# victorca25/traiNNer

Measured on AMD Instinct MI355X. Metric: HR images/sec (G+D step), ESRGAN x4 128->512, higher is better.
Workload: dtype f32 (bf16x3)

## Files before the change

trainner_amd/csrc/conv_sweep.hip:

```cpp
#include <stddef.h>
#include <string.h>
#include <type_traits>
#include <utility>
#include "conv_body.h"
#include "conv_epilogue.h"
#include "conv_handoff.h"

namespace {

constexpr int SW_TH = 8, SW_TW = 32, SW_HT = SW_TH + 2, SW_WT = SW_TW + 2;
constexpr int SW_ROW = TNR_X3_ROW;
constexpr int SW_A_ROWS = SW_HT * SW_WT;
constexpr int SW_A_ALLOC_ROWS = 384;
constexpr int SW_A_FLOATS = SW_A_ALLOC_ROWS * SW_ROW;
constexpr int SW_UNIT_FLOATS = 32 * SW_ROW;
constexpr int SW_SLOT_UNITS = 9;
constexpr int SW_SLOT_FLOATS = SW_SLOT_UNITS * SW_UNIT_FLOATS;
constexpr int SW_RING = 3;
constexpr size_t SW_LDS_BYTES = (size_t)(2 * SW_A_FLOATS + SW_RING * SW_SLOT_FLOATS) * sizeof(float);
constexpr int SW_NPASS = 9, SW_NSTAGE = 5, SW_NTILE = 6;
constexpr int SW_A_IT = (SW_A_ROWS * 4 + 511) / 512;
constexpr int SW_B_PIECES = (SW_SLOT_UNITS * 3 + 7) / 8;
static_assert(SW_LDS_BYTES <= 160 * 1024, "one sweep workgroup per CU");

// ... 773 lines not shown
            constexpr int S = decltype(sc)::value;
            SW_T(t_e0);
            const ConvK a = sweep_stage(S);
            const __amdgpu_buffer_rsrc_t y_rs =
                __builtin_amdgcn_make_buffer_rsrc(a.y, 0, (int)((unsigned)a.N * a.Ho * a.Wo * a.y_ct * 4u), 0x00020000);
            if constexpr (S < 4) {
                f32x16 t[2][1];
                t[0][0] = acc[0][S];
                t[1][0] = acc[1][S];
                conv_epilogue_dpp<TNR_CONV_3x3, SW_TW, 1, 2, true, 8, false>(a, t, 0, n, ty0, tx0, 0, wave, li, half, y_rs);
            } else {
                f32x16 t[2][2];
#pragma unroll
                for (int m = 0; m < 2; ++m) {
                    t[m][0] = acc[m][4];
                    t[m][1] = acc[m][5];
                }
                conv_epilogue_dpp<TNR_CONV_3x3, SW_TW, 2, 2, true, 8>(a, t, 0, n, ty0, tx0, 0, wave, li, half, y_rs);
            }
            pend_tile = tile;
            pend_value = c.base + (unsigned)S + 1u;
            pend_age = 0;
            { SW_T(t_e1); SW_ADD(8, t_e1 - t_e0); }
        };
        auto sync = [&](auto sc) __attribute__((always_inline)) {
            constexpr int sl = decltype(sc)::value;
            slot_sync((sl + 1) % SW_RING);
        };
        auto item_step = [&](auto ic, auto kc) __attribute__((always_inline)) {
            if (has_next) item_step_buf(ic, kc, (e + 1) & 1);
        };

        sw_static_for<0, P::NPASS>([&](auto pc) __attribute__((always_inline)) {
            constexpr int p = decltype(pc)::value;
            const int nchunks = sw_nchunks(p, c.nck0), ch_lo = sw_ch_lo(p, c.nck0);
#pragma unroll 1
            for (int ck = 0; ck < nchunks; ++ck) {
                slot_sync(1);
                if constexpr (!sw_apass(p) && !(DIRECT && S4D_EPI_AFTER)) {
                    if (ck == 0) epilogue_of(std::integral_constant<int, sw_phase(p)>{});
                }
                const bool last_ck = ck + 1 == nchunks;
                has_next = !(last_ck && p == P::NPASS - 1);
                int ch_keep = 0;
                if (has_next) {
                    int ch_next = ch_lo + 16 * (ck + 1);
                    if (last_ck) {
                        ch_next = sw_ch_lo(p + 1 < P::NPASS ? p + 1 : p, c.nck0);
                        if constexpr (p + 1 < P::NPASS && sw_apass(p + 1)) {
                            const ChainWait w{c.progress, c.base + (unsigned)sw_phase(p + 1), n, ty, tx, c.tiles_x, c.tiles_y, c.err,
                                              &pend_tile, pend_value};
                            SW_T(t_w0);
                            w();
                            { SW_T(t_w1); SW_ADD(1, t_w1 - t_w0); }
                        }
                    }
                    if constexpr (!(DIRECT && S4D_ALOAD_ALWAYS)) {
                        SW_T(t_al0);
                        a_load(ch_next);
                        { SW_T(t_al1); SW_ADD(2, t_al1 - t_al0); }
                    } else {
                        ch_keep = ch_next;
                    }
                }
                if constexpr (DIRECT && S4D_ALOAD_ALWAYS) {
                    SW_T(t_al0);
                    a_load(ch_keep, has_next);
                    { SW_T(t_al1); SW_ADD(2, t_al1 - t_al0); }
                }
                const float *sa = s_a + (e & 1) * SW_A_FLOATS;
                SW_T(t_c0);
                if constexpr (AMP) {
                    auto item1 = [&](auto ic) __attribute__((always_inline)) {
                        if (has_next) a_item1(ic, (e + 1) & 1);
                    };
                    amp4_chunk<P::j0(p), P::nj(p)>(acc, sa, apix0, half, item1, fbq, b_fetch1);
                } else {
                    sweep4_chunk<P::j0(p), P::nj(p), DIRECT>(acc, sa, s_b_lane, apix0, half, sync, item_step, dma_step, tick, fbr, b_fetch);
                }
                { SW_T(t_c1); SW_ADD(6, t_c1 - t_c0); SW_ADD(15, 1ull); SW_ADD(9 + (P::nj(p) == 3 ? 0 : (P::nj(p) == 2 ? 1 : 2)), t_c1 - t_c0); }
                ++e;
            }
            if constexpr (DIRECT && S4D_EPI_AFTER && sw_apass(p) && p + 1 < P::NPASS) {
                epilogue_of(std::integral_constant<int, sw_phase(p)>{});
            }
        });
        epilogue_of(std::integral_constant<int, P::NSTAGE - 1>{});
    }
    asm volatile("s_waitcnt vmcnt(0)" ::: "memory");
    __syncthreads();
    if (pend_tile >= 0 && tid == 0) __hip_atomic_store(c.progress + pend_tile, pend_value, __ATOMIC_RELAXED, __HIP_MEMORY_SCOPE_AGENT);
    if (tid == 0 && atomicAdd(c.disp + 8, 1u) == (unsigned)g - 1u) {
#pragma unroll
        for (int i = 0; i < 9; ++i) __hip_atomic_store(c.disp + i, 0u, __ATOMIC_RELAXED, __HIP_MEMORY_SCOPE_AGENT);
    }
#ifdef SW_TIMELINE
    if (tid == 0) {
        tl[14] = __builtin_amdgcn_s_memtime() - tl_begin;
        for (int i = 0; i < 16; ++i) atomicAdd(&sw_tl[i], tl[i]);
        for (int i = 0; i < 16; ++i) atomicAdd(&sw_tl2[i], tl2[i]);
    }
#endif
}

struct D4K {
    ConvK a;
    const float *wq;
    int wq_bytes;
    int nck;
    int tiles_x, tiles_y, ncb, tiles;
};

struct D4PackK {
    const float *wp;
    int KinP, KoutP, nck, ncb, units;
    int shuffle;
    float *out;
};

__global__ void __launch_bounds__(256) d4_pack_kernel(const D4PackK a) {
    const int g = blockIdx.x * 256 + threadIdx.x;
    const int unit = g >> 6, r = (g >> 1) & 31, h = g & 1;
    if (unit >= a.units) return;
    const int per_cb = a.nck * 18;
    const int cb = unit / per_cb, rem = unit - cb * per_cb;
    const int ck = rem / 18, tj = rem - ck * 18, tap = tj >> 1, j = tj & 1;
    int co = cb * 64 + j * 32 + r;
    if (a.shuffle == 2) {
        const int nfc = a.KoutP >> 2;
        co = (co % nfc) * 4 + co / nfc;
    }
    const float *src = a.wp + ((size_t)tap * a.KoutP + co) * a.KinP + 16 * ck + 8 * h;
    const f32x4 q0 = *reinterpret_cast<const f32x4 *>(src), q1 = *reinterpret_cast<const f32x4 *>(src + 4);
    tnr_bf16x8 pl[3];
    tnr_split_bf16x3(q0, q1, pl);
    float *dst = a.out + (size_t)unit * SW_UNIT_FLOATS + (h * 32 + r) * 4;
#pragma unroll
    for (int k = 0; k < 3; ++k) *reinterpret_cast<tnr_bf16x8 *>(dst + k * 256) = pl[k];
}

template <int OCC, bool AMP = false, bool PS = false>
__global__ void __launch_bounds__(256, OCC) conv3x3_d4_kernel(const D4K c) {
    extern __shared__ __attribute__((aligned(16))) float smem[];
    float *s_a = smem;
    const int tid = threadIdx.x;
    const int wave = __builtin_amdgcn_readfirstlane(tid >> 6), lane = tid & 63, li = lane & 31, half = lane >> 5;
    const ConvK &a = c.a;
    const __amdgpu_buffer_rsrc_t x_rs =
        __builtin_amdgcn_make_buffer_rsrc(const_cast<float *>(a.x), 0, (int)((unsigned)a.N * a.H * a.W * a.x_ct * 4u), 0x00020000);
    const __amdgpu_buffer_rsrc_t w_rs = __builtin_amdgcn_make_buffer_rsrc(const_cast<float *>(c.wq), 0, c.wq_bytes, 0x00020000);
    const __amdgpu_buffer_rsrc_t y_rs =
        __builtin_amdgcn_make_buffer_rsrc(a.y, 0, (int)((unsigned)a.N * a.Ho * a.Wo * a.y_ct * 4u), 0x00020000);
    const int apix0[2] = {(2 * wave) * SW_WT + li, (2 * wave + 1) * SW_WT + li};

    for (int tile = blockIdx.x; tile < c.tiles; tile += gridDim.x) {
        const int cb = tile % c.ncb;
        int rest = tile / c.ncb;
        const int tx = rest % c.tiles_x;
        rest /= c.tiles_x;
        const int ty = rest % c.tiles_y, n = rest / c.tiles_y;
        const int ty0 = ty * SW_TH, tx0 = tx * SW_TW;
        int in_off[S4_A_IT], a_dst[S4_A_IT];
#pragma unroll
        for (int it = 0; it < S4_A_IT; ++it) {
            const int i = tid + it * 256, row = i >> 2, q = i & 3;
            const int hr = row / SW_WT, hc = row - hr * SW_WT;
            int Y = ty0 + hr - 1, X = tx0 + hc - 1;
            if (a.reflect) {
                Y = Y == -1 ? 1 : (Y == a.H ? a.H - 2 : Y);
                X = X == -1 ? 1 : (X == a.W ? a.W - 2 : X);
            }
            const bool in = (row < SW_A_ROWS) & (Y >= 0) & (Y < a.H) & (X >= 0) & (X < a.W);
            in_off[it] = in ? (((n * a.H + Y) * a.W + X) * a.x_ct + a.x_co + q * 4) : -1;
            a_dst[it] = row * SW_ROW + 4 * ((q >> 1) ^ ((row >> TNR_X3_SWZ) & 1)) + 2 * (q & 1);
        }
        f32x4 rin[S4_A_IT];
        auto a_load = [&](int ch, bool valid) __attribute__((always_inline)) {
#pragma unroll
            for (int it = 0; it < S4_A_IT; ++it) {
                const unsigned bo = (valid && in_off[it] >= 0) ? (unsigned)(in_off[it] + ch) * 4u : 0xfffffff0u;
                rin[it] = __builtin_bit_cast(f32x4, __builtin_amdgcn_raw_buffer_load_b128(x_rs, (int)bo, 0, 0));
            }
        };
        tnr_bf16x4 ih, im, il;
        f32x4 ir;
        auto item_step_buf = [&](auto ic, auto kc, int buf) __attribute__((always_inline)) {
            constexpr int it = decltype(ic)::value, k = decltype(kc)::value;
            if constexpr (k == 0) {
                tnr_pk_level(rin[it], ih, ir);
            } else if constexpr (k == 1) {
                const f32x4 r1 = ir;
                tnr_pk_level(r1, im, ir);
            } else {
                if constexpr (k == 2) {
                    const tnr_f32x2 a2 = {ir[0], ir[1]}, b2 = {ir[2], ir[3]};
                    il = __builtin_bit_cast(tnr_bf16x4, tnr_f32x2{__builtin_bit_cast(float, __builtin_convertvector(a2, tnr_bf16x2)),
                                                                __builtin_bit_cast(float, __builtin_convertvector(b2, tnr_bf16x2))});
                }
                float *dst = s_a + buf * SW_A_FLOATS + a_dst[it] + 8 * (k - 2);
                *reinterpret_cast<tnr_f32x2 *>(dst) = __builtin_bit_cast(tnr_f32x2, k == 2 ? ih : (k == 3 ? im : il));
            }
        };
        f32x16 acc[2][SW_NTILE];
#pragma unroll
        for (int m = 0; m < 2; ++m)
#pragma unroll
            for (int j = 0; j < 2; ++j)
#pragma unroll
                for (int r = 0; r < 16; ++r) acc[m][j][r] = 0.f;

        a_load(0, true);
        __syncthreads();
        tnr_bf16x8 fbr[3][3];
        int bq = cb * c.nck * 18;
        auto b_fetch = [&](auto rc, int sp) __attribute__((always_inline)) {
            constexpr int r = decltype(rc)::value;
            fbr[r][sp] = __builtin_bit_cast(tnr_bf16x8, __builtin_amdgcn_raw_buffer_load_b128(w_rs, lane * 16, (bq * 3 + sp) * 1024, 0));
            if (sp == 2) ++bq;
        };
        tnr_bf16x8 fbq[9];
        auto b_fetch1 = [&](auto rc) __attribute__((always_inline)) {
            constexpr int r = decltype(rc)::value;
            fbq[r] = __builtin_bit_cast(tnr_bf16x8, __builtin_amdgcn_raw_buffer_load_b128(w_rs, lane * 16, bq * 3072, 0));
            ++bq;
        };
        auto a_item1 = [&](auto ic, int buf) __attribute__((always_inline)) {
            constexpr int it = decltype(ic)::value;
            const tnr_bf16x4 h = __builtin_convertvector(rin[it], tnr_bf16x4);
            *reinterpret_cast<tnr_f32x2 *>(s_a + buf * SW_A_FLOATS + a_dst[it]) = __builtin_bit_cast(tnr_f32x2, h);
        };
        if constexpr (AMP) {
            sw_static_for<0, 8>([&](auto rc) __attribute__((always_inline)) { b_fetch1(rc); });
            sw_static_for<0, S4_A_IT>([&](auto ic) __attribute__((always_inline)) { a_item1(ic, 0); });
        } else {
#pragma unroll
            for (int sp = 0; sp < 3; ++sp) b_fetch(std::integral_constant<int, 0>{}, sp);
#pragma unroll
            for (int sp = 0; sp < 3; ++sp) b_fetch(std::integral_constant<int, 1>{}, sp);
            sw_static_for<0, S4_A_IT>([&](auto ic) __attribute__((always_inline)) {
                sw_static_for<0, 5>([&](auto kc) __attribute__((always_inline)) { item_step_buf(ic, kc, 0); });
            });
        }
        bool has_next = false;
        int e = 0;
        auto item_step = [&](auto ic, auto kc) __attribute__((always_inline)) {
            if (has_next) item_step_buf(ic, kc, (e + 1) & 1);
        };
        auto nop1 = [&](auto) __attribute__((always_inline)) {};
        auto nop0 = [&]() __attribute__((always_inline)) {};
        auto tick = [&](int, unsigned long long) __attribute__((always_inline)) {};
#pragma unroll 1
        for (int ck = 0; ck < c.nck; ++ck) {
            asm volatile("s_waitcnt lgkmcnt(0)\n\ts_barrier" ::: "memory");
            has_next = ck + 1 < c.nck;
            a_load(16 * (ck + 1), has_next);
            if constexpr (AMP) {
                auto item1 = [&](auto ic) __attribute__((always_inline)) {
                    if (has_next) a_item1(ic, (e + 1) & 1);
                };
                amp4_chunk<0, 2>(acc, s_a + (e & 1) * SW_A_FLOATS, apix0, half, item1, fbq, b_fetch1);
            } else {
                sweep4_chunk<0, 2, true>(acc, s_a + (e & 1) * SW_A_FLOATS, nullptr, apix0, half, nop1, item_step, nop0, tick, fbr, b_fetch);
            }
            ++e;
        }
        f32x16 t[2][2];
#pragma unroll
        for (int m = 0; m < 2; ++m) {
            t[m][0] = acc[m][0];
            t[m][1] = acc[m][1];
        }
        if constexpr (PS) {
            ConvK ap = a;
            const int nfb = c.ncb >> 2, sub = cb / nfb;
            ap.Cout = a.Cout >> 2;
            ap.Ho = 2 * a.Ho;
            ap.Wo = 2 * a.Wo;
            ap.bias = a.bias != nullptr ? a.bias + sub : nullptr;
            conv_epilogue_dpp<TNR_DGRAD_4x4_S2, SW_TW, 2, 2, false, (OCC == 1 ? 8 : 1), false, 4>(ap, t, cb - sub * nfb, n, ty0, tx0, sub, wave, li, half, y_rs);
        } else {
            conv_epilogue_dpp<TNR_CONV_3x3, SW_TW, 2, 2, false, (OCC == 1 ? 8 : 1)>(a, t, cb, n, ty0, tx0, 0, wave, li, half, y_rs);
        }
    }
}

constexpr int S2_TAPS = 4, S2_NU = S2_TAPS * 2, S2_RING = 4;
struct S2K {
    ConvK a;
    const float *wq;
    int wq_bytes;
    int nck;
    int tiles_x, tiles_y, ncb, tiles;
};
struct S2PackK {
    const float *wp;
    int KinP, KoutP, nck, ncb, units, dgrad;
    float *out;
};

__global__ void __launch_bounds__(256) s2_pack_kernel(const S2PackK a) {
    const int g = blockIdx.x * 256 + threadIdx.x;
    const int unit = g >> 6, r = (g >> 1) & 31, h = g & 1;
    if (unit >= a.units) return;
    const int j = unit & 1, tap = (unit >> 1) & 3;
    int rest = unit >> 3;
    const float *src;
    if (a.dgrad) {
        const int ck = rest % a.nck;
        rest /= a.nck;
        const int cb = rest % a.ncb, par = rest / a.ncb;
        src = a.wp + (((size_t)par * 4 + tap) * a.KoutP + cb * 64 + j * 32 + r) * a.KinP + 16 * ck + 8 * h;
    } else {
        const int ck = rest % a.nck;
        rest /= a.nck;
        const int pp = rest & 3, cb = rest >> 2;
        src = a.wp + ((size_t)tap * a.KoutP + cb * 64 + j * 32 + r) * (4 * a.KinP) + pp * a.KinP + 16 * ck + 8 * h;
    }
    const f32x4 q0 = *reinterpret_cast<const f32x4 *>(src), q1 = *reinterpret_cast<const f32x4 *>(src + 4);
    tnr_bf16x8 pl[3];
    tnr_split_bf16x3(q0, q1, pl);
    float *dst = a.out + (size_t)unit * SW_UNIT_FLOATS + (h * 32 + r) * 4;
#pragma unroll
    for (int k = 0; k < 3; ++k) *reinterpret_cast<tnr_bf16x8 *>(dst + k * 256) = pl[k];
}

template <bool AMP, class Item, class BFetch>
__device__ __forceinline__ void tap4_chunk(f32x16 (&acc)[2][2], const float *sa, const int (&aaddr)[2][4], Item &&item_step,
                                           tnr_bf16x8 (&fbr)[S2_RING][3], BFetch &&b_fetch) {
    constexpr int TA[6] = {0, 2, 1, 0, 1, 0}, TB[6] = {2, 0, 1, 1, 0, 0};
    tnr_bf16x8 fa[2][2][3];
    auto read_a = [&](auto tc, int m, int sp) __attribute__((always_inline)) {
        constexpr int t = decltype(tc)::value;
        fa[t & 1][m][sp] = *reinterpret_cast<const tnr_bf16x8 *>(sa + aaddr[m][t] + 8 * sp);
    };
#pragma unroll
    for (int k = 0; k < (AMP ? 2 : 6); ++k) read_a(std::integral_constant<int, 0>{}, AMP ? k : k / 3, AMP ? 0 : k % 3);
    sw_static_for<0, S2_NU>([&](auto uc) __attribute__((always_inline)) {
        constexpr int u = decltype(uc)::value, t = u >> 1, jj = u & 1;
        constexpr bool NEXT_TAP = jj == 1 && t + 1 < S2_TAPS;
        constexpr int ITEM = u - (S2_NU - 6);
        __builtin_amdgcn_sched_barrier(0);
        if constexpr (AMP) {
            sw_static_for<0, 2>([&](auto mc) __attribute__((always_inline)) {
                constexpr int m = decltype(mc)::value;
                acc[m][jj] = __builtin_amdgcn_mfma_f32_32x32x16_bf16(fa[t & 1][m][0], fbr[u % S2_RING][0], acc[m][jj], 0, 0, 0);
                if constexpr (m == 0) b_fetch(std::integral_constant<int, (u + 3) % S2_RING>{}, 0);
                if constexpr (NEXT_TAP) read_a(std::integral_constant<int, (t + 1 < S2_TAPS ? t + 1 : t)>{}, m, 0);
                if constexpr (m == 1 && ITEM >= 0) item_step(std::integral_constant<int, (ITEM >= 0 ? ITEM : 0)>{}, std::integral_constant<int, -1>{});
                __builtin_amdgcn_sched_barrier(0);
            });
        } else {
            sw_static_for<0, 12>([&](auto ic) __attribute__((always_inline)) {
                constexpr int i = decltype(ic)::value, p = i / 2, m = i % 2;
                acc[m][jj] = __builtin_amdgcn_mfma_f32_32x32x16_bf16(fa[t & 1][m][TA[p]], fbr[u % S2_RING][TB[p]], acc[m][jj], 0, 0, 0);
                if constexpr (i < 3) b_fetch(std::integral_constant<int, (u + 3) % S2_RING>{}, i);
                if constexpr (NEXT_TAP && i >= 3 && i < 9) read_a(std::integral_constant<int, (t + 1 < S2_TAPS ? t + 1 : t)>{}, (i - 3) / 3, (i - 3) % 3);
                if constexpr (ITEM >= 0 && i >= 4 && i < 9) item_step(std::integral_constant<int, (ITEM >= 0 ? ITEM : 0)>{}, std::integral_constant<int, (i >= 4 && i < 9 ? i - 4 : 0)>{});
                __builtin_amdgcn_sched_barrier(0);
            });
        }
    });
}

template <int MODE, bool AMP>
__global__ void __launch_bounds__(256, 2) conv_s2_d4_kernel(const S2K c) {
    constexpr bool DG = MODE == TNR_DGRAD_4x4_S2;
    constexpr int HT = DG ? SW_HT : SW_TH + 1, WT = DG ? SW_WT : SW_TW + 1, ROWS = HT * WT;
    constexpr int A_IT = (ROWS * 4 + 255) / 256;
    static_assert(A_IT <= 6 && A_IT * 256 <= SW_A_ALLOC_ROWS * 4, "staging plan");
    extern __shared__ __attribute__((aligned(16))) float smem[];
    float *s_a = smem;
    const int tid = threadIdx.x;
    const int wave = __builtin_amdgcn_readfirstlane(tid >> 6), lane = tid & 63, li = lane & 31, half = lane >> 5;
    const ConvK &a = c.a;
    const __amdgpu_buffer_rsrc_t x_rs =
        __builtin_amdgcn_make_buffer_rsrc(const_cast<float *>(a.x), 0, (int)((unsigned)a.N * a.H * a.W * a.x_ct * 4u), 0x00020000);
    const __amdgpu_buffer_rsrc_t w_rs = __builtin_amdgcn_make_buffer_rsrc(const_cast<float *>(c.wq), 0, c.wq_bytes, 0x00020000);
    const __amdgpu_buffer_rsrc_t y_rs =
        __builtin_amdgcn_make_buffer_rsrc(a.y, 0, (int)((unsigned)a.N * a.Ho * a.Wo * a.y_ct * 4u), 0x00020000);
    const int nchunks = DG ? c.nck : 4 * c.nck;

    for (int tile = blockIdx.x; tile < c.tiles; tile += gridDim.x) {
        int rest = tile;
        const int cb = rest % c.ncb;
        rest /= c.ncb;
        int par = 0;
        if constexpr (DG) {
            par = rest & 3;
            rest >>= 2;
        }
        const int tx = rest % c.tiles_x;
        rest /= c.tiles_x;
        const int ty = rest % c.tiles_y, n = rest / c.tiles_y;
        const int ty0 = ty * SW_TH, tx0 = tx * SW_TW;
        const int py = par >> 1, px = par & 1;
        int aaddr[2][4];
#pragma unroll
        for (int m = 0; m < 2; ++m)
#pragma unroll
            for (int t = 0; t < 4; ++t) {
                const int pos_y = DG ? 1 + py - (t >> 1) : (t >> 1), pos_x = DG ? 1 + px - (t & 1) : (t & 1);
                const int pp = (2 * wave + m + pos_y) * WT + li + pos_x;
                aaddr[m][t] = pp * SW_ROW + 4 * (half ^ ((pp >> TNR_X3_SWZ) & 1));
            }
        int in_off[A_IT], a_dst[A_IT];
        auto plan = [&](int pp) __attribute__((always_inline)) {
#pragma unroll
            for (int it = 0; it < A_IT; ++it) {
                const int i = tid + it * 256, row = i >> 2, q = i & 3;
                const int hr = row / WT, hc = row - hr * WT;
                const int Y = DG ? ty0 + hr - 1 : 2 * (ty0 + hr) - 1 + (pp >> 1), X = DG ? tx0 + hc - 1 : 2 * (tx0 + hc) - 1 + (pp & 1);
                const bool in = (row < ROWS) & (Y >= 0) & (Y < a.H) & (X >= 0) & (X < a.W);
                in_off[it] = in ? (((n * a.H + Y) * a.W + X) * a.x_ct + a.x_co + q * 4) : -1;
                a_dst[it] = row * SW_ROW + 4 * ((q >> 1) ^ ((row >> TNR_X3_SWZ) & 1)) + 2 * (q & 1);
            }
        };
        plan(0);
        f32x4 rin[A_IT];
        auto a_load = [&](int ch, bool valid) __attribute__((always_inline)) {
#pragma unroll
            for (int it = 0; it < A_IT; ++it) {
                const unsigned bo = (valid && in_off[it] >= 0) ? (unsigned)(in_off[it] + ch) * 4u : 0xfffffff0u;
                rin[it] = __builtin_bit_cast(f32x4, __builtin_amdgcn_raw_buffer_load_b128(x_rs, (int)bo, 0, 0));
            }
        };
        tnr_bf16x4 ih, im, il;
        f32x4 ir;
        auto item_step_buf = [&](auto ic, auto kc, int buf) __attribute__((always_inline)) {
            constexpr int it = decltype(ic)::value, k = decltype(kc)::value;
            if constexpr (it < A_IT) {
                if constexpr (k < 0) {
                    const tnr_bf16x4 hh = __builtin_convertvector(rin[it], tnr_bf16x4);
                    *reinterpret_cast<tnr_f32x2 *>(s_a + buf * SW_A_FLOATS + a_dst[it]) = __builtin_bit_cast(tnr_f32x2, hh);
                } else if constexpr (k == 0) {
                    tnr_pk_level(rin[it], ih, ir);
                } else if constexpr (k == 1) {
                    const f32x4 r1 = ir;
                    tnr_pk_level(r1, im, ir);
                } else {
                    if constexpr (k == 2) {
                        const tnr_f32x2 a2 = {ir[0], ir[1]}, b2 = {ir[2], ir[3]};
                        il = __builtin_bit_cast(tnr_bf16x4, tnr_f32x2{__builtin_bit_cast(float, __builtin_convertvector(a2, tnr_bf16x2)),
                                                                    __builtin_bit_cast(float, __builtin_convertvector(b2, tnr_bf16x2))});
                    }
                    float *dst = s_a + buf * SW_A_FLOATS + a_dst[it] + 8 * (k - 2);
                    *reinterpret_cast<tnr_f32x2 *>(dst) = __builtin_bit_cast(tnr_f32x2, k == 2 ? ih : (k == 3 ? im : il));
                }
            }
        };
        f32x16 acc[2][2];
#pragma unroll
        for (int m = 0; m < 2; ++m)
#pragma unroll
            for (int j = 0; j < 2; ++j)
#pragma unroll
                for (int r = 0; r < 16; ++r) acc[m][j][r] = 0.f;

        a_load(0, true);
        __syncthreads();
        tnr_bf16x8 fbr[S2_RING][3];
        int bq = (DG ? (par * c.ncb + cb) * c.nck : cb * 4 * c.nck) * S2_NU;
        auto b_fetch = [&](auto rc, int sp) __attribute__((always_inline)) {
            constexpr int r = decltype(rc)::value;
            if constexpr (AMP) {
                fbr[r][0] = __builtin_bit_cast(tnr_bf16x8, __builtin_amdgcn_raw_buffer_load_b128(w_rs, lane * 16, bq * 3072, 0));
                ++bq;
            } else {
                fbr[r][sp] = __builtin_bit_cast(tnr_bf16x8, __builtin_amdgcn_raw_buffer_load_b128(w_rs, lane * 16, (bq * 3 + sp) * 1024, 0));
                if (sp == 2) ++bq;
            }
        };
        sw_static_for<0, 3>([&](auto rc) __attribute__((always_inline)) {
#pragma unroll
            for (int sp = 0; sp < (AMP ? 1 : 3); ++sp) b_fetch(rc, sp);
        });
        sw_static_for<0, 6>([&](auto ic) __attribute__((always_inline)) {
            if constexpr (AMP) item_step_buf(ic, std::integral_constant<int, -1>{}, 0);
            else sw_static_for<0, 5>([&](auto kc) __attribute__((always_inline)) { item_step_buf(ic, kc, 0); });
        });
        bool has_next = false;
        int e = 0;
        auto item_step = [&](auto ic, auto kc) __attribute__((always_inline)) {
            if (has_next) item_step_buf(ic, kc, (e + 1) & 1);
        };
#pragma unroll 1
        for (int ck = 0; ck < nchunks; ++ck) {
            asm volatile("s_waitcnt lgkmcnt(0)\n\ts_barrier" ::: "memory");
            has_next = ck + 1 < nchunks;
            int ch_next = 16 * (ck + 1);
            if constexpr (!DG) {
                const int nx = ck + 1, ppn = nx / c.nck;
                ch_next = 16 * (nx - ppn * c.nck);
                if (has_next && ppn != ck / c.nck) plan(ppn);
            }
            a_load(ch_next, has_next);
            tap4_chunk<AMP>(acc, s_a + (e & 1) * SW_A_FLOATS, aaddr, item_step, fbr, b_fetch);
            ++e;
        }
        f32x16 t2[2][2];
#pragma unroll
        for (int m = 0; m < 2; ++m) {
            t2[m][0] = acc[m][0];
            t2[m][1] = acc[m][1];
        }
        conv_epilogue_dpp<MODE, SW_TW, 2, 2, false, 1>(a, t2, cb, n, ty0, tx0, par, wave, li, half, y_rs);
    }
}

bool s2_ok(const tnr_conv_desc *d) {
    if (d->mode != TNR_CONV_4x4_S2 && d->mode != TNR_DGRAD_4x4_S2) return false;
    const bool dg = d->mode == TNR_DGRAD_4x4_S2;
    const int tw = dg ? d->W : d->Wo, th = dg ? d->H : d->Ho;
    return (d->mma == TNR_MMA_BF16X3 || d->mma == TNR_MMA_BF16) && d->pad_mode == 0 && d->shuffle == 0 && (d->Cout % 64) == 0 && d->KoutP == d->Cout &&
           d->Cin == d->KinP && (d->Cin % 16) == 0 && d->Cin >= 32 && tw >= 32 && th >= 8 &&
           (dg ? (d->Ho == 2 * d->H && d->Wo == 2 * d->W) : (d->H == 2 * d->Ho && d->W == 2 * d->Wo)) &&
           buffers_addressable(*d) &&
           (int64_t)(d->Cout / 64) * (d->Cin / 16) * 4 * S2_NU * SW_UNIT_FLOATS * (int64_t)sizeof(float) < (1LL << 31);
}

bool d4_ok(const tnr_conv_desc *d) {
    if (d->shuffle != 0 && !(d->shuffle == 2 && (d->Cout % 256) == 0 && d->r1.ptr == nullptr && d->r2.ptr == nullptr && d->m.ptr == nullptr &&
                             d->noise_pos == 0 && d->pad_mode == 0 && (d->y.ctot % 4) == 0 &&
                             (int64_t)d->N * d->H * d->W * 4 * d->y.ctot < (1LL << 30)))
        return false;
    return d->mode == TNR_CONV_3x3 && (d->mma == TNR_MMA_BF16X3 || d->mma == TNR_MMA_BF16) && (d->pad_mode == 0 || (d->pad_mode == 1 && d->H >= 2 && d->W >= 2)) &&
           (d->Cout % 64) == 0 && d->KoutP == d->Cout &&
           d->Cin == d->KinP && (d->Cin % 16) == 0 && d->Cin >= 32 && d->Ho == d->H && d->Wo == d->W && d->W >= 32 && d->H >= 8 &&
           buffers_addressable(*d) &&
           (int64_t)(d->Cout / 64) * (d->Cin / 16) * 18 * SW_UNIT_FLOATS * (int64_t)sizeof(float) < (1LL << 31);
}

bool sweep_pattern(const tnr_conv_desc *st, int n, const char **why) {
    auto no = [&](const char *w) { if (why) *why = w; return false; };
    if (st == nullptr || (n != SW_NSTAGE && n != SW4_NSTAGE)) return no("not 5 (or 4) stages");
    if (n == SW4_NSTAGE && st[0].mma != TNR_MMA_BF16X3) return no("the four-stage form exists in bf16x3 only");
    const tnr_conv_desc &d0 = st[0];
    if (d0.Cin < 32 || (d0.Cin % 16) != 0) return no("block input channels must be a multiple of 16, >= 32");
    for (int i = 0; i < n; ++i) {
        const tnr_conv_desc &d = st[i];
        if (d.mode != TNR_CONV_3x3 || (d.mma != TNR_MMA_BF16X3 && d.mma != TNR_MMA_BF16) || d.mma != d0.mma || d.pad_mode != 0)
            return no("stage is not a zero-padded 3x3 in bf16x3 (or all stages with bf16 operands)");
        if (d.N != d0.N || d.H != d0.H || d.W != d0.W || d.Ho != d0.H || d.Wo != d0.W) return no("pixel grids differ");
        if (d.x.ptr != d0.x.ptr || d.x.ctot != d0.x.ctot || d.x.coff != d0.x.coff) return no("stages read different buffers");
        if (d.Cin != d0.Cin + 32 * i || d.KinP != d.Cin) return no("input channels do not grow by 32 per stage");
        if (d.Cout != (i < 4 ? 32 : 64) || d.KoutP != d.Cout) return no("output channels are not 32, 32, 32, 32, 64");
        if (i < 4 && (d.y.ptr != d0.x.ptr || d.y.ctot != d0.x.ctot || d.y.coff != d0.x.coff + d.Cin)) return no("stage output is not the next channel group");
        if (!views_aligned(d)) return no("x / y / r1 / r2 / mask views must be 4-channel aligned");
        if (d.noise_pos < 0 || d.noise_pos > 2 || (i < 4 && d.noise_pos != 0)) return no("the noise multiplier belongs to the last stage");
        if (!buffers_addressable(d)) return no("buffer above 4 GiB");
        if (!d.x.ptr || !d.y.ptr || !d.wp) return no("null pointer");
    }
    const tnr_conv_desc &dl = st[n - 1];
    if (n == SW_NSTAGE && dl.y.ptr == d0.x.ptr && dl.y.coff < d0.x.coff + dl.Cin && dl.y.coff + dl.Cout > d0.x.coff) return no("last stage overwrites its own input");
    return true;
}

int sweep_form() {
    static const int form = [] {
        const char *w = getenv("TNR_SWEEP_WAVES"), *f = getenv("TNR_SWEEP_FORM");
        if (w && atoi(w) == 8) return 8;
        return (f && f[0] == 'd' && f[1] == 'm') ? 4 : 5;
    }();
    return form;
}
constexpr size_t S4D_LDS_BYTES = (size_t)(2 * SW_A_FLOATS) * sizeof(float);

int sweep_cus() {
    static int cus = 0;
    tnr_kernel_setup(&cus, "conv_sweep", {{conv_sweep_kernel, SW_LDS_BYTES}, {conv_sweep4_kernel<false>, SW_LDS_BYTES},
                                          {conv_sweep4_kernel<true>, S4D_LDS_BYTES}, {conv_sweep4_kernel<true, true>, S4D_LDS_BYTES},
                                          {conv_sweep4_kernel<true, false, SwPlan4>, S4D_LDS_BYTES}});
    return cus;
}

int sweep_pack_args(const char *who, const tnr_conv_desc *stages, int n, void *image, int64_t image_bytes, SweepPackK &a) {
    a.nck0 = stages[0].Cin / 16;
    a.ns = n;
    a.units = sw_total_units(a.nck0, n);
    a.direct = sweep_form() == 5;
    TNR_REQUIRE((int64_t)a.units * SW_UNIT_FLOATS * (int64_t)sizeof(float) <= image_bytes, "%s: image buffer too small", who);
    TNR_REQUIRE(n == SW_NSTAGE || a.direct, "%s: four stages run in the direct four-wave form only", who);
    for (int i = 0; i < SW_NSTAGE; ++i) {
        const tnr_conv_desc &d = stages[i < n ? i : n - 1];
        a.wp[i] = d.wp;
        a.KinP[i] = d.KinP;
        a.KoutP[i] = d.KoutP;
    }
    a.out = static_cast<float *>(image);
    return TNR_OK;
}

}

#ifdef SW_TIMELINE
extern "C" int tnr_debug_sweep_units(unsigned long long *out16, int reset) {
    if (out16 != nullptr && hipMemcpyFromSymbol(out16, HIP_SYMBOL(sw_tl2), sizeof(sw_tl2)) != hipSuccess) return TNR_ELAUNCH;
    if (reset) {
        unsigned long long z[16] = {0, 0, 0, 0, 0, 0, 0, 0, 0, 0, 0, 0, 0, 0, 0, 0};
        if (hipMemcpyToSymbol(HIP_SYMBOL(sw_tl2), z, sizeof(z)) != hipSuccess) return TNR_ELAUNCH;
    }
    return TNR_OK;
}
extern "C" int tnr_debug_sweep_timeline(unsigned long long *out16, int reset) {
    if (out16 != nullptr && hipMemcpyFromSymbol(out16, HIP_SYMBOL(sw_tl), sizeof(sw_tl)) != hipSuccess) return TNR_ELAUNCH;
    if (reset) {
        unsigned long long z[16] = {0, 0, 0, 0, 0, 0, 0, 0, 0, 0, 0, 0, 0, 0, 0, 0};
        if (hipMemcpyToSymbol(HIP_SYMBOL(sw_tl), z, sizeof(z)) != hipSuccess) return TNR_ELAUNCH;
    }
    return TNR_OK;
}
#endif

extern "C" int64_t tnr_conv_sweep_image_bytes(const tnr_conv_desc *stages, int32_t n) {
    if (stages == nullptr || !sweep_pattern(stages, n, nullptr)) return 0;
    if ((stages[0].mma == TNR_MMA_BF16 || n == SW4_NSTAGE) && sweep_form() != 5) return 0;
    const int cus = sweep_cus();
    const int tpi = tnr_cdiv(stages[0].W, SW_TW) * tnr_cdiv(stages[0].H, SW_TH);
    if (cus < 1 || tpi > cus) return 0;
    return (int64_t)sw_total_units(stages[0].Cin / 16, n) * SW_UNIT_FLOATS * (int64_t)sizeof(float);
}

extern "C" int tnr_conv_sweep_pack(const tnr_conv_desc *stages, int32_t n, void *image, int64_t image_bytes, void *stream) {
    const char *why = "";
    TNR_REQUIRE(stages != nullptr && image != nullptr && sweep_pattern(stages, n, &why), "conv_sweep_pack: not a sweepable dense block (%s)", why);
    SweepPackK a;
    if (const int rc = sweep_pack_args("conv_sweep_pack", stages, n, image, image_bytes, a)) return rc;
    hipLaunchKernelGGL(sweep_pack_kernel, dim3((unsigned)tnr_cdiv(a.units * 64, 256)), dim3(256), 0, (hipStream_t)stream, a);
    return tnr_check_launch("conv_sweep_pack");
}

static_assert(sizeof(SweepPackK) <= sizeof(((tnr_sweep_pack_item *)nullptr)->opaque), "tnr_sweep_pack_item holds the pack kernel's arguments");

extern "C" int tnr_conv_sweep_pack_item(const tnr_conv_desc *stages, int32_t n, void *image, int64_t image_bytes, tnr_sweep_pack_item *item) {
    const char *why = "";
    TNR_REQUIRE(stages != nullptr && image != nullptr && item != nullptr && sweep_pattern(stages, n, &why),
                "conv_sweep_pack_item: not a sweepable dense block (%s)", why);
    SweepPackK a;
    if (const int rc = sweep_pack_args("conv_sweep_pack_item", stages, n, image, image_bytes, a)) return rc;
    memset(item, 0, sizeof(*item));
    memcpy(item->opaque, &a, sizeof(a));
    item->units = a.units;
    return TNR_OK;
}

extern "C" int tnr_conv_sweep_pack_batch(const tnr_sweep_pack_item *items_dev, int32_t n, int32_t max_units, void *stream) {
    TNR_REQUIRE(items_dev != nullptr && n >= 1 && n <= 65535 && max_units >= 1, "conv_sweep_pack_batch: bad arguments");
    static_assert(sizeof(tnr_sweep_pack_item) % 8 == 0, "table stride");
    hipLaunchKernelGGL(sweep_pack_batch_strided_kernel, dim3((unsigned)tnr_cdiv(max_units * 64, 256), (unsigned)n), dim3(256), 0, (hipStream_t)stream, items_dev);
    return tnr_check_launch("conv_sweep_pack_batch");
}

extern "C" int tnr_conv_sweep(const tnr_conv_desc *stages, int32_t n, const void *image, uint32_t *ws, int64_t ws_bytes, uint32_t epoch,
                              void *stream) {
    const char *why = "";
    TNR_REQUIRE(stages != nullptr && image != nullptr && ws != nullptr && sweep_pattern(stages, n, &why),
                "conv_sweep: not a sweepable dense block (%s)", why);
    const tnr_conv_desc &d0 = stages[0];
    TNR_REQUIRE(tnr_conv_chain_workspace_bytes(&d0) <= ws_bytes, "conv_sweep: workspace too small");
    const int cus = sweep_cus();
    if (cus < 1) return TNR_ELAUNCH;
    SweepK c;
    c.nck0 = d0.Cin / 16;
    c.tiles_x = tnr_cdiv(d0.W, SW_TW);
    c.tiles_y = tnr_cdiv(d0.H, SW_TH);
    c.tpi = c.tiles_x * c.tiles_y;
    c.tiles = c.tpi * d0.N;
    TNR_REQUIRE(c.tpi <= cus, "conv_sweep: the %d tiles of an image exceed the %d co-resident workgroups", c.tpi, cus);
    c.progress = ws;
    c.err = tnr_fault_word_or(ws + ws_bytes / 4 - 1);
    static const int nxcd = [] { const char *e = getenv("TNR_SWEEP_DISPENSERS"); return e ? atoi(e) : 1; }();
    c.nxcd = nxcd == 1 ? 1 : 8;
    c.disp = ws + (ws_bytes / 4 - 1 - 4 - CH_CU_KEYS - CH_SWEEP_WORDS);
    c.base = epoch * (uint32_t)(TNR_CHAIN_MAX + 2);
    c.wq = static_cast<const float *>(image);
    c.wq_bytes = sw_total_units(c.nck0, n) * SW_UNIT_FLOATS * (int)sizeof(float);
    for (int i = 0; i < SW_NSTAGE; ++i) {
        const tnr_conv_desc *d = &stages[i < n ? i : n - 1];
        ConvK &k = c.st[i] = conv_k_from_desc(*d);
        k.tiles_x = c.tiles_x; k.tiles_y = c.tiles_y; k.ncb = d->KoutP / 32;
    }
    const int per_round = (cus / c.tpi) * c.tpi;
    const int grid = c.tiles < per_round ? c.tiles : per_round;
    const int form = sweep_form();
    if (n == SW4_NSTAGE) {
        TNR_REQUIRE(form == 5, "conv_sweep: four stages run in the direct four-wave form only");
        hipLaunchKernelGGL((conv_sweep4_kernel<true, false, SwPlan4>), dim3((unsigned)grid), dim3(256), S4D_LDS_BYTES, (hipStream_t)stream, c);
        return tnr_check_launch("conv_sweep");
    }
    if (stages[0].mma == TNR_MMA_BF16) {
        TNR_REQUIRE(form == 5, "conv_sweep: bf16 operands (use_amp) run in the direct four-wave form only");
        hipLaunchKernelGGL((conv_sweep4_kernel<true, true>), dim3((unsigned)grid), dim3(256), S4D_LDS_BYTES, (hipStream_t)stream, c);
        return tnr_check_launch("conv_sweep");
    }
    if (form == 8) hipLaunchKernelGGL(conv_sweep_kernel, dim3((unsigned)grid), dim3(512), SW_LDS_BYTES, (hipStream_t)stream, c);
    else if (form == 4) hipLaunchKernelGGL(conv_sweep4_kernel<false>, dim3((unsigned)grid), dim3(256), SW_LDS_BYTES, (hipStream_t)stream, c);
    else hipLaunchKernelGGL(conv_sweep4_kernel<true>, dim3((unsigned)grid), dim3(256), S4D_LDS_BYTES, (hipStream_t)stream, c);
    return tnr_check_launch("conv_sweep");
}

extern "C" int64_t tnr_conv_wq_bytes(const tnr_conv_desc *d) {
    if (d != nullptr && s2_ok(d)) return (int64_t)(d->Cout / 64) * (d->Cin / 16) * 4 * S2_NU * SW_UNIT_FLOATS * (int64_t)sizeof(float);
    if (d == nullptr || !d4_ok(d)) return 0;
    return (int64_t)(d->Cout / 64) * (d->Cin / 16) * 18 * SW_UNIT_FLOATS * (int64_t)sizeof(float);
}

extern "C" int tnr_conv_wq_pack(const tnr_conv_desc *d, void *image, int64_t image_bytes, void *stream) {
    if (d != nullptr && image != nullptr && d->wp != nullptr && s2_ok(d)) {
        S2PackK a;
        a.wp = d->wp; a.KinP = d->KinP; a.KoutP = d->KoutP; a.nck = d->Cin / 16; a.ncb = d->Cout / 64;
        a.dgrad = d->mode == TNR_DGRAD_4x4_S2;
        a.units = a.ncb * 4 * a.nck * S2_NU;
        TNR_REQUIRE((int64_t)a.units * SW_UNIT_FLOATS * (int64_t)sizeof(float) <= image_bytes, "conv_wq_pack: image buffer too small");
        a.out = static_cast<float *>(image);
        hipLaunchKernelGGL(s2_pack_kernel, dim3((unsigned)tnr_cdiv(a.units * 64, 256)), dim3(256), 0, (hipStream_t)stream, a);
        return tnr_check_launch("conv_wq_pack (four-tap form)");
    }
    TNR_REQUIRE(d != nullptr && image != nullptr && d->wp != nullptr && d4_ok(d), "conv_wq_pack: the launch cannot use a pre-split weight stream");
    D4PackK a;
    a.wp = d->wp; a.KinP = d->KinP; a.KoutP = d->KoutP; a.nck = d->Cin / 16; a.ncb = d->Cout / 64;
    a.units = a.ncb * a.nck * 18;
    a.shuffle = d->shuffle;
    TNR_REQUIRE((int64_t)a.units * SW_UNIT_FLOATS * (int64_t)sizeof(float) <= image_bytes, "conv_wq_pack: image buffer too small");
    a.out = static_cast<float *>(image);
    hipLaunchKernelGGL(d4_pack_kernel, dim3((unsigned)tnr_cdiv(a.units * 64, 256)), dim3(256), 0, (hipStream_t)stream, a);
    return tnr_check_launch("conv_wq_pack");
}

int tnr_launch_conv_s2_d4(const tnr_conv_desc *d, void *stream) {
    if (!s2_ok(d) || d->wq == nullptr || d->wq_bytes < tnr_conv_wq_bytes(d) || d->noise_pos != 0) return 1;
    static int cus = 0;
    if (const int rc = tnr_kernel_setup(&cus, "conv_s2_d4", {{conv_s2_d4_kernel<TNR_CONV_4x4_S2, false>, S4D_LDS_BYTES}, {conv_s2_d4_kernel<TNR_CONV_4x4_S2, true>, S4D_LDS_BYTES},
                                                             {conv_s2_d4_kernel<TNR_DGRAD_4x4_S2, false>, S4D_LDS_BYTES}, {conv_s2_d4_kernel<TNR_DGRAD_4x4_S2, true>, S4D_LDS_BYTES}}))
        return rc;
    const bool dg = d->mode == TNR_DGRAD_4x4_S2;
    S2K c;
    if (!stream_k_from_desc(c, *d, tnr_conv_wq_bytes(d), SW_TW, SW_TH, dg ? 4 : 1)) return 1;
    const unsigned grid = (unsigned)(c.tiles < 2 * cus ? c.tiles : 2 * cus);
    const bool amp = d->mma == TNR_MMA_BF16;
    if (dg) {
        if (amp) hipLaunchKernelGGL((conv_s2_d4_kernel<TNR_DGRAD_4x4_S2, true>), dim3(grid), dim3(256), S4D_LDS_BYTES, (hipStream_t)stream, c);
        else hipLaunchKernelGGL((conv_s2_d4_kernel<TNR_DGRAD_4x4_S2, false>), dim3(grid), dim3(256), S4D_LDS_BYTES, (hipStream_t)stream, c);
    } else {
        if (amp) hipLaunchKernelGGL((conv_s2_d4_kernel<TNR_CONV_4x4_S2, true>), dim3(grid), dim3(256), S4D_LDS_BYTES, (hipStream_t)stream, c);
        else hipLaunchKernelGGL((conv_s2_d4_kernel<TNR_CONV_4x4_S2, false>), dim3(grid), dim3(256), S4D_LDS_BYTES, (hipStream_t)stream, c);
    }
    return tnr_check_launch("conv_s2_d4");
}

int tnr_launch_conv3x3_d4(const tnr_conv_desc *d, void *stream) {
    if (!d4_ok(d) || d->wq == nullptr || d->wq_bytes < tnr_conv_wq_bytes(d) || d->noise_pos < 0 || d->noise_pos > 2) return 1;
    static int occ = [] { const char *e = getenv("TNR_D4_OCC"); return e ? atoi(e) : 2; }();
    static int cus = 0;
    if (const int rc = tnr_kernel_setup(&cus, "conv3x3_d4", {{conv3x3_d4_kernel<1>, S4D_LDS_BYTES}, {conv3x3_d4_kernel<2>, S4D_LDS_BYTES}, {conv3x3_d4_kernel<2, true>, S4D_LDS_BYTES},
                                                             {conv3x3_d4_kernel<2, false, true>, S4D_LDS_BYTES}, {conv3x3_d4_kernel<2, true, true>, S4D_LDS_BYTES}}))
        return rc;
    D4K c;
    if (!stream_k_from_desc(c, *d, tnr_conv_wq_bytes(d), SW_TW, SW_TH, 1)) return 1;
    const int slots = cus * (occ == 1 ? 1 : 2);
    const int grid = c.tiles < slots ? c.tiles : slots;
    if (d->shuffle == 2) {
        const unsigned g2 = (unsigned)(c.tiles < 2 * cus ? c.tiles : 2 * cus);
        if (d->mma == TNR_MMA_BF16) hipLaunchKernelGGL((conv3x3_d4_kernel<2, true, true>), dim3(g2), dim3(256), S4D_LDS_BYTES, (hipStream_t)stream, c);
        else hipLaunchKernelGGL((conv3x3_d4_kernel<2, false, true>), dim3(g2), dim3(256), S4D_LDS_BYTES, (hipStream_t)stream, c);
        return tnr_check_launch("conv3x3_d4 (pixel-shuffle store)");
    }
    if (d->mma == TNR_MMA_BF16) hipLaunchKernelGGL((conv3x3_d4_kernel<2, true>), dim3((unsigned)(c.tiles < 2 * cus ? c.tiles : 2 * cus)), dim3(256), S4D_LDS_BYTES, (hipStream_t)stream, c);
    else if (occ == 1) hipLaunchKernelGGL(conv3x3_d4_kernel<1>, dim3((unsigned)grid), dim3(256), S4D_LDS_BYTES, (hipStream_t)stream, c);
    else hipLaunchKernelGGL(conv3x3_d4_kernel<2>, dim3((unsigned)grid), dim3(256), S4D_LDS_BYTES, (hipStream_t)stream, c);
    return tnr_check_launch("conv3x3_d4");
}
```

Baseline: 75.54.

## Pair output parities in stride-2 data-gradient conv to share staged input tile

Adds a paired form of the 4x4 stride-2 data-gradient kernel in which each workgroup computes two x-parities for one y-parity. Both parities read from a single staged input tile, which halves the number of tiles and cuts redundant input staging. The weight pack kernel gains a matching layout that interleaves the two parities' taps. In the non-AMP path the input loads are spread through the MFMA schedule, and a remapped epilogue writes the interleaved outputs. The change uses more accumulator registers and a more complex schedule, and it is on by default behind an environment toggle.

```diff
diff --git a/trainner_amd/csrc/conv_sweep.hip b/trainner_amd/csrc/conv_sweep.hip
--- a/trainner_amd/csrc/conv_sweep.hip
+++ b/trainner_amd/csrc/conv_sweep.hip
@@ -1099,10 +1099,18 @@
     const int g = blockIdx.x * 256 + threadIdx.x;
     const int unit = g >> 6, r = (g >> 1) & 31, h = g & 1;
     if (unit >= a.units) return;
-    const int j = unit & 1, tap = (unit >> 1) & 3;
-    int rest = unit >> 3;
+    const int j = unit & 1;
+    int tap = (unit >> 1) & 3, rest = unit >> 3;
     const float *src;
-    if (a.dgrad) {
+    if (a.dgrad == 2) {
+        const int g = (unit >> 1) & 7;
+        tap = g >> 1;
+        rest = unit >> 4;
+        const int ck = rest % a.nck;
+        rest /= a.nck;
+        const int cb = rest % a.ncb, par = 2 * (rest / a.ncb) + 1 - (g & 1);
+        src = a.wp + (((size_t)par * 4 + tap) * a.KoutP + cb * 64 + j * 32 + r) * a.KinP + 16 * ck + 8 * h;
+    } else if (a.dgrad) {
         const int ck = rest % a.nck;
         rest /= a.nck;
         const int cb = rest % a.ncb, par = rest / a.ncb;
@@ -1159,10 +1167,68 @@
     });
 }
 
-template <int MODE, bool AMP>
+constexpr int S2P_NU = 2 * S2_NU;
+constexpr int S2P_LOAD[5] = {0, 3, 5, 8, 10}, S2P_ITEM[5] = {5, 8, 10, 13, 15};
+template <bool AMP>
+constexpr int s2p_find(const int (&tab)[5], int u) {
+    for (int k = 0; k < 5; ++k)
+        if (!AMP && tab[k] == u) return k;
+    return -1;
+}
+template <bool AMP, int A_IT, class Item, class BFetch>
+__device__ __forceinline__ void tap4_pair_chunk(f32x16 (&acc)[4][2], const float *sa, const int row0, const int half, Item &&item_step,
+                                                tnr_bf16x8 (&fbr)[S2_RING][3], BFetch &&b_fetch) {
+    constexpr int TA[6] = {0, 2, 1, 0, 1, 0}, TB[6] = {2, 0, 1, 1, 0, 0};
+    constexpr int GP[9] = {0, 1, 1, 2, 3, 4, 4, 5, 6};
+    tnr_bf16x8 fa[2][2][3];
+    int row = row0;
+    asm volatile("" : "+v"(row));
+    auto read_a = [&](auto pc, int m, int sp) __attribute__((always_inline)) {
+        constexpr int p = decltype(pc)::value;
+        const int pp = row + (m + 1 - p / 3) * SW_WT + 2 - p % 3;
+        fa[sp == 0 ? (p & 1) : 0][m][sp] = *reinterpret_cast<const tnr_bf16x8 *>(sa + pp * SW_ROW + 4 * (half ^ ((pp >> TNR_X3_SWZ) & 1)) + 8 * sp);
+    };
+#pragma unroll
+    for (int k = 0; k < (AMP ? 2 : 6); ++k) read_a(std::integral_constant<int, 0>{}, AMP ? k : k / 3, AMP ? 0 : k % 3);
+    sw_static_for<0, S2P_NU>([&](auto uc) __attribute__((always_inline)) {
+        constexpr int u = decltype(uc)::value, g = u >> 1, jj = u & 1, px = 1 - (g & 1), p = GP[g];
+        constexpr bool NEXT_POS = jj == 1 && GP[g + 1] != p && p + 1 < 6;
+        constexpr int PN = p + 1 < 6 ? p + 1 : p;
+        static_assert(A_IT == 5, "staging schedule");
+        constexpr int ITEM = AMP ? u - (S2P_NU - A_IT) : s2p_find<AMP>(S2P_ITEM, u), LOAD = s2p_find<AMP>(S2P_LOAD, u);
+        __builtin_amdgcn_sched_barrier(0);
+        if constexpr (AMP) {
+            sw_static_for<0, 2>([&](auto mc) __attribute__((always_inline)) {
+                constexpr int m = decltype(mc)::value;
+                acc[2 * m + px][jj] = __builtin_amdgcn_mfma_f32_32x32x16_bf16(fa[p & 1][m][0], fbr[u % S2_RING][0], acc[2 * m + px][jj], 0, 0, 0);
+                if constexpr (m == 0) b_fetch(std::integral_constant<int, (u + 3) % S2_RING>{}, 0);
+                if constexpr (NEXT_POS) read_a(std::integral_constant<int, PN>{}, m, 0);
+                if constexpr (m == 1 && ITEM >= 0) item_step(std::integral_constant<int, (ITEM >= 0 ? ITEM : 0)>{}, std::integral_constant<int, -1>{});
+                __builtin_amdgcn_sched_barrier(0);
+            });
+        } else {
+            sw_static_for<0, 12>([&](auto ic) __attribute__((always_inline)) {
+                constexpr int i = decltype(ic)::value, q = i / 2, m = i % 2;
+                acc[2 * m + px][jj] = __builtin_amdgcn_mfma_f32_32x32x16_bf16(fa[TA[q] == 0 ? (p & 1) : 0][m][TA[q]], fbr[u % S2_RING][TB[q]], acc[2 * m + px][jj], 0, 0, 0);
+                if constexpr (i < 3) b_fetch(std::integral_constant<int, (u + 3) % S2_RING>{}, i);
+                if constexpr (NEXT_POS) {
+                    if constexpr (i == 3 || i == 4) read_a(std::integral_constant<int, PN>{}, i - 3, 2);
+                    if constexpr (i == 5 || i == 6) read_a(std::integral_constant<int, PN>{}, i - 5, 0);
+                    if constexpr (i == 9 || i == 10) read_a(std::integral_constant<int, PN>{}, i - 9, 1);
+                }
+                if constexpr (LOAD >= 0 && i == 11) item_step(std::integral_constant<int, (LOAD >= 0 ? LOAD : 0)>{}, std::integral_constant<int, -2>{});
+                if constexpr (ITEM >= 0 && i >= 4 && i < 9) item_step(std::integral_constant<int, (ITEM >= 0 ? ITEM : 0)>{}, std::integral_constant<int, (i >= 4 && i < 9 ? i - 4 : 0)>{});
+                __builtin_amdgcn_sched_barrier(0);
+            });
+        }
+    });
+}
+
+template <int MODE, bool AMP, bool PAIR = false>
 __global__ void __launch_bounds__(256, 2) conv_s2_d4_kernel(const S2K c) {
     constexpr bool DG = MODE == TNR_DGRAD_4x4_S2;
-    constexpr int HT = DG ? SW_HT : SW_TH + 1, WT = DG ? SW_WT : SW_TW + 1, ROWS = HT * WT;
+    static_assert(DG || !PAIR, "the pair form is the data-gradient's");
+    constexpr int HT = DG && !PAIR ? SW_HT : SW_TH + 1, WT = DG ? SW_WT : SW_TW + 1, ROWS = HT * WT;
     constexpr int A_IT = (ROWS * 4 + 255) / 256;
     static_assert(A_IT <= 6 && A_IT * 256 <= SW_A_ALLOC_ROWS * 4, "staging plan");
     extern __shared__ __attribute__((aligned(16))) float smem[];
@@ -1182,7 +1248,10 @@
         const int cb = rest % c.ncb;
         rest /= c.ncb;
         int par = 0;
-        if constexpr (DG) {
+        if constexpr (PAIR) {
+            par = 2 * (rest & 1);
+            rest >>= 1;
+        } else if constexpr (DG) {
             par = rest & 3;
             rest >>= 2;
         }
@@ -1202,24 +1271,28 @@
             }
         int in_off[A_IT], a_dst[A_IT];
         auto plan = [&](int pp) __attribute__((always_inline)) {
+            int tid_p = tid;
+            if constexpr (PAIR) asm volatile("" : "+v"(tid_p));
 #pragma unroll
             for (int it = 0; it < A_IT; ++it) {
-                const int i = tid + it * 256, row = i >> 2, q = i & 3;
+                const int i = tid_p + it * 256, row = i >> 2, q = i & 3;
                 const int hr = row / WT, hc = row - hr * WT;
-                const int Y = DG ? ty0 + hr - 1 : 2 * (ty0 + hr) - 1 + (pp >> 1), X = DG ? tx0 + hc - 1 : 2 * (tx0 + hc) - 1 + (pp & 1);
+                const int Y = DG ? ty0 + hr - 1 + (PAIR ? py : 0) : 2 * (ty0 + hr) - 1 + (pp >> 1), X = DG ? tx0 + hc - 1 : 2 * (tx0 + hc) - 1 + (pp & 1);
                 const bool in = (row < ROWS) & (Y >= 0) & (Y < a.H) & (X >= 0) & (X < a.W);
                 in_off[it] = in ? (((n * a.H + Y) * a.W + X) * a.x_ct + a.x_co + q * 4) : -1;
                 a_dst[it] = row * SW_ROW + 4 * ((q >> 1) ^ ((row >> TNR_X3_SWZ) & 1)) + 2 * (q & 1);
+                if constexpr (PAIR) a_dst[it] = a_dst[0] + it * 64 * SW_ROW;
             }
         };
         plan(0);
         f32x4 rin[A_IT];
+        auto a_load1 = [&](int it, int ch, bool valid) __attribute__((always_inline)) {
+            const unsigned bo = (valid && in_off[it] >= 0) ? (unsigned)(in_off[it] + ch) * 4u : 0xfffffff0u;
+            rin[it] = __builtin_bit_cast(f32x4, __builtin_amdgcn_raw_buffer_load_b128(x_rs, (int)bo, 0, 0));
+        };
         auto a_load = [&](int ch, bool valid) __attribute__((always_inline)) {
 #pragma unroll
-            for (int it = 0; it < A_IT; ++it) {
-                const unsigned bo = (valid && in_off[it] >= 0) ? (unsigned)(in_off[it] + ch) * 4u : 0xfffffff0u;
-                rin[it] = __builtin_bit_cast(f32x4, __builtin_amdgcn_raw_buffer_load_b128(x_rs, (int)bo, 0, 0));
-            }
+            for (int it = 0; it < A_IT; ++it) a_load1(it, ch, valid);
         };
         tnr_bf16x4 ih, im, il;
         f32x4 ir;
@@ -1245,9 +1318,9 @@
                 }
             }
         };
-        f32x16 acc[2][2];
-#pragma unroll
-        for (int m = 0; m < 2; ++m)
+        f32x16 acc[PAIR ? 4 : 2][2];
+#pragma unroll
+        for (int m = 0; m < (PAIR ? 4 : 2); ++m)
 #pragma unroll
             for (int j = 0; j < 2; ++j)
 #pragma unroll
@@ -1256,7 +1329,7 @@
         a_load(0, true);
         __syncthreads();
         tnr_bf16x8 fbr[S2_RING][3];
-        int bq = (DG ? (par * c.ncb + cb) * c.nck : cb * 4 * c.nck) * S2_NU;
+        int bq = (PAIR ? (py * c.ncb + cb) * c.nck * 2 : (DG ? (par * c.ncb + cb) * c.nck : cb * 4 * c.nck)) * S2_NU;
         auto b_fetch = [&](auto rc, int sp) __attribute__((always_inline)) {
             constexpr int r = decltype(rc)::value;
             if constexpr (AMP) {
@@ -1276,32 +1349,53 @@
             else sw_static_for<0, 5>([&](auto kc) __attribute__((always_inline)) { item_step_buf(ic, kc, 0); });
         });
         bool has_next = false;
-        int e = 0;
+        int e = 0, ch_next = 0;
         auto item_step = [&](auto ic, auto kc) __attribute__((always_inline)) {
-            if (has_next) item_step_buf(ic, kc, (e + 1) & 1);
+            if constexpr (decltype(kc)::value == -2) a_load1(decltype(ic)::value, ch_next, has_next);
+            else if (has_next) item_step_buf(ic, kc, (e + 1) & 1);
         };
 #pragma unroll 1
         for (int ck = 0; ck < nchunks; ++ck) {
             asm volatile("s_waitcnt lgkmcnt(0)\n\ts_barrier" ::: "memory");
             has_next = ck + 1 < nchunks;
-            int ch_next = 16 * (ck + 1);
+            ch_next = 16 * (ck + 1);
             if constexpr (!DG) {
                 const int nx = ck + 1, ppn = nx / c.nck;
                 ch_next = 16 * (nx - ppn * c.nck);
                 if (has_next && ppn != ck / c.nck) plan(ppn);
             }
-            a_load(ch_next, has_next);
-            tap4_chunk<AMP>(acc, s_a + (e & 1) * SW_A_FLOATS, aaddr, item_step, fbr, b_fetch);
+            if constexpr (!PAIR || AMP) a_load(ch_next, has_next);
+            if constexpr (PAIR) tap4_pair_chunk<AMP, A_IT>(acc, s_a + (e & 1) * SW_A_FLOATS, 2 * wave * SW_WT + li, half, item_step, fbr, b_fetch);
+            else tap4_chunk<AMP>(acc, s_a + (e & 1) * SW_A_FLOATS, aaddr, item_step, fbr, b_fetch);
             ++e;
         }
-        f32x16 t2[2][2];
-#pragma unroll
-        for (int m = 0; m < 2; ++m) {
-            t2[m][0] = acc[m][0];
-            t2[m][1] = acc[m][1];
-        }
-        conv_epilogue_dpp<MODE, SW_TW, 2, 2, false, 1>(a, t2, cb, n, ty0, tx0, par, wave, li, half, y_rs);
-    }
+        if constexpr (PAIR) {
+            ConvK ap = a;
+            ap.th_space = a.Ho;
+            ap.tw_space = a.Wo;
+            int li_e = li, half_e = half;
+            asm volatile("" : "+v"(li_e), "+v"(half_e));
+            conv_epilogue_dpp_map<TNR_CONV_3x3, SW_TW, 2, 4, false, 1>(ap, acc, cb, n, 2 * ty0 + py, 2 * tx0, 0, li_e, half_e, y_rs,
+                                                                     [&](int mi, int row, int &rr, int &cc) __attribute__((always_inline)) {
+                                                                         const int p = (wave * 2 + (mi >> 1)) * 32 + row, r = p / SW_TW;
+                                                                         rr = 2 * r;
+                                                                         cc = 2 * (p - r * SW_TW) + (mi & 1);
+                                                                     });
+        } else {
+            f32x16 t2[2][2];
+#pragma unroll
+            for (int m = 0; m < 2; ++m) {
+                t2[m][0] = acc[m][0];
+                t2[m][1] = acc[m][1];
+            }
+            conv_epilogue_dpp<MODE, SW_TW, 2, 2, false, 1>(a, t2, cb, n, ty0, tx0, par, wave, li, half, y_rs);
+        }
+    }
+}
+
+bool s2_pairs() {
+    static const bool pairs = [] { const char *e = getenv("TNR_S2_PAIRS"); return e == nullptr || atoi(e) != 0; }();
+    return pairs;
 }
 
 bool s2_ok(const tnr_conv_desc *d) {
@@ -1505,7 +1599,7 @@
     if (d != nullptr && image != nullptr && d->wp != nullptr && s2_ok(d)) {
         S2PackK a;
         a.wp = d->wp; a.KinP = d->KinP; a.KoutP = d->KoutP; a.nck = d->Cin / 16; a.ncb = d->Cout / 64;
-        a.dgrad = d->mode == TNR_DGRAD_4x4_S2;
+        a.dgrad = d->mode == TNR_DGRAD_4x4_S2 ? (s2_pairs() ? 2 : 1) : 0;
         a.units = a.ncb * 4 * a.nck * S2_NU;
         TNR_REQUIRE((int64_t)a.units * SW_UNIT_FLOATS * (int64_t)sizeof(float) <= image_bytes, "conv_wq_pack: image buffer too small");
         a.out = static_cast<float *>(image);
@@ -1527,14 +1621,18 @@
     if (!s2_ok(d) || d->wq == nullptr || d->wq_bytes < tnr_conv_wq_bytes(d) || d->noise_pos != 0) return 1;
     static int cus = 0;
     if (const int rc = tnr_kernel_setup(&cus, "conv_s2_d4", {{conv_s2_d4_kernel<TNR_CONV_4x4_S2, false>, S4D_LDS_BYTES}, {conv_s2_d4_kernel<TNR_CONV_4x4_S2, true>, S4D_LDS_BYTES},
-                                                             {conv_s2_d4_kernel<TNR_DGRAD_4x4_S2, false>, S4D_LDS_BYTES}, {conv_s2_d4_kernel<TNR_DGRAD_4x4_S2, true>, S4D_LDS_BYTES}}))
+                                                             {conv_s2_d4_kernel<TNR_DGRAD_4x4_S2, false>, S4D_LDS_BYTES}, {conv_s2_d4_kernel<TNR_DGRAD_4x4_S2, true>, S4D_LDS_BYTES},
+                                                             {conv_s2_d4_kernel<TNR_DGRAD_4x4_S2, false, true>, S4D_LDS_BYTES}, {conv_s2_d4_kernel<TNR_DGRAD_4x4_S2, true, true>, S4D_LDS_BYTES}}))
         return rc;
-    const bool dg = d->mode == TNR_DGRAD_4x4_S2;
+    const bool dg = d->mode == TNR_DGRAD_4x4_S2, pair = dg && s2_pairs();
     S2K c;
-    if (!stream_k_from_desc(c, *d, tnr_conv_wq_bytes(d), SW_TW, SW_TH, dg ? 4 : 1)) return 1;
+    if (!stream_k_from_desc(c, *d, tnr_conv_wq_bytes(d), SW_TW, SW_TH, pair ? 2 : (dg ? 4 : 1))) return 1;
     const unsigned grid = (unsigned)(c.tiles < 2 * cus ? c.tiles : 2 * cus);
     const bool amp = d->mma == TNR_MMA_BF16;
-    if (dg) {
+    if (pair) {
+        if (amp) hipLaunchKernelGGL((conv_s2_d4_kernel<TNR_DGRAD_4x4_S2, true, true>), dim3(grid), dim3(256), S4D_LDS_BYTES, (hipStream_t)stream, c);
+        else hipLaunchKernelGGL((conv_s2_d4_kernel<TNR_DGRAD_4x4_S2, false, true>), dim3(grid), dim3(256), S4D_LDS_BYTES, (hipStream_t)stream, c);
+    } else if (dg) {
         if (amp) hipLaunchKernelGGL((conv_s2_d4_kernel<TNR_DGRAD_4x4_S2, true>), dim3(grid), dim3(256), S4D_LDS_BYTES, (hipStream_t)stream, c);
         else hipLaunchKernelGGL((conv_s2_d4_kernel<TNR_DGRAD_4x4_S2, false>), dim3(grid), dim3(256), S4D_LDS_BYTES, (hipStream_t)stream, c);
     } else {
```

New measurement: 75.71, median of 6. About the same (+0.2%).
